# amathislab/HOISDF

Measured on AMD Instinct MI355X. Metric: samples/sec (img + 2048 SDF queries) fwd+bwd at 1/2/4/8 MI355X, higher is better.
Workload: dtype f32 (emulated contractions, f32 accumulate, f16x2 form: operands as scaled hi + lo f16 pieces x 3 products - 22 operand bits, one power-of-two scale per ROW of a linear layer's row operand, per (sample, head) of the attention operands, per weight matrix; the attention backward's dS as three pieces x

## Files before the change

hoisdf_amd/csrc/bnact.hip:

```cpp
#include "common.h"

namespace hoisdf {
namespace {
typedef float f32x4 __attribute__((ext_vector_type(4)));
constexpr int BN_T = 256;

struct Geom { int tpr, rpi; };
__host__ __device__ __forceinline__ Geom geom(int C) { Geom g; g.tpr = C >> 3; g.rpi = BN_T / g.tpr; return g; }
__host__ __device__ __forceinline__ int chunk_of(int C) { return C % 64 == 0 ? 64 : C % 32 == 0 ? 32 : C % 16 == 0 ? 16 : 8; }

__device__ __forceinline__ void ld8(const float* p, float (&v)[8]) {
  const f32x4 a = *reinterpret_cast<const f32x4*>(p), b = *reinterpret_cast<const f32x4*>(p + 4);
  v[0] = a[0]; v[1] = a[1]; v[2] = a[2]; v[3] = a[3]; v[4] = b[0]; v[5] = b[1]; v[6] = b[2]; v[7] = b[3];
}
__device__ __forceinline__ void st8(float* p, const float (&v)[8]) {
  *reinterpret_cast<f32x4*>(p) = f32x4{v[0], v[1], v[2], v[3]};
  *reinterpret_cast<f32x4*>(p + 4) = f32x4{v[4], v[5], v[6], v[7]};
}

__device__ __forceinline__ void block_partials(const float (&s)[16], float* red, int tpr, int rpi, int chunk, float* __restrict__ part) {
  const int tid = threadIdx.x;
#pragma unroll
  for (int j = 0; j < 16; ++j) red[j * BN_T + tid] = s[j];
  __syncthreads();
  float* dst = part + ((size_t)blockIdx.y * gridDim.x + blockIdx.x) * 2 * chunk;
  for (int o = tid; o < 2 * chunk; o += BN_T) {
    const int pl = o / chunk, ch = o - pl * chunk;
    const int j = pl * 8 + (ch & 7), t0 = ch >> 3;
    float a = 0.f;
    for (int g = 0; g < rpi; ++g) a += red[j * BN_T + g * tpr + t0];
    dst[o] = a;
  }
}
__device__ __forceinline__ void sum_partials(const float* __restrict__ part, int S, int chunk, double* dred, double& a1, double& a2) {
  const int tid = threadIdx.x;
  const int lanes = chunk >> 1;
  const int G = BN_T / lanes, lane = tid % lanes, g = tid / lanes;
  const f32x4* src = reinterpret_cast<const f32x4*>(part + (size_t)blockIdx.x * S * 2 * chunk) + lane;
  double acc[4] = {0.0, 0.0, 0.0, 0.0};
  int sl = g;
  for (; sl + 3 * G < S; sl += 4 * G) {
    f32x4 v[4];
#pragma unroll
    for (int u = 0; u < 4; ++u) v[u] = src[(size_t)(sl + u * G) * lanes];
#pragma unroll
    for (int u = 0; u < 4; ++u)
#pragma unroll
      for (int i = 0; i < 4; ++i) acc[i] += (double)v[u][i];
  }
  for (; sl < S; sl += G) {
    const f32x4 v = src[(size_t)sl * lanes];
#pragma unroll
    for (int i = 0; i < 4; ++i) acc[i] += (double)v[i];
  }
#pragma unroll
  for (int i = 0; i < 4; ++i) dred[(g * lanes + lane) * 4 + i] = acc[i];
  __syncthreads();
  a1 = 0.0; a2 = 0.0;
  if (tid < chunk) {
    const int l1 = tid >> 2, l2 = (chunk >> 2) + (tid >> 2), i = tid & 3;
    for (int g2 = 0; g2 < G; ++g2) { a1 += dred[(g2 * lanes + l1) * 4 + i]; a2 += dred[(g2 * lanes + l2) * 4 + i]; }
  }
}

__global__ __launch_bounds__(BN_T) void bn_stats_kernel(const float* __restrict__ x, long ldx, long M, int C, long rows_per_block,
                                                        float* __restrict__ part) {
  __shared__ __attribute__((aligned(16))) float red[16 * BN_T];
  const int chunk = chunk_of(C), tpr = chunk >> 3, rpi = BN_T / tpr;
  const int tid = threadIdx.x, cg = tid % tpr, rg = tid / tpr;
  const int c0 = blockIdx.y * chunk + 8 * cg;
  const long r0 = (long)blockIdx.x * rows_per_block, r1 = r0 + rows_per_block < M ? r0 + rows_per_block : M;
  float s[16], sh[8];
#pragma unroll
  for (int j = 0; j < 16; ++j) s[j] = 0.f;
  ld8(x + c0, sh);
  {
    const long step = rpi;
    long r = r0 + rg;
    for (; r + 3 * step < r1; r += 4 * step) {
      float v[4][8];
#pragma unroll
      for (int u = 0; u < 4; ++u) ld8(x + (r + u * step) * ldx + c0, v[u]);
#pragma unroll
      for (int u = 0; u < 4; ++u)
#pragma unroll
        for (int j = 0; j < 8; ++j) { const float d = v[u][j] - sh[j]; s[j] += d; s[8 + j] = __builtin_fmaf(d, d, s[8 + j]); }
    }
    for (; r < r1; r += step) {
      float v[8];
      ld8(x + r * ldx + c0, v);
#pragma unroll
      for (int j = 0; j < 8; ++j) { const float d = v[j] - sh[j]; s[j] += d; s[8 + j] = __builtin_fmaf(d, d, s[8 + j]); }
    }
  }
  block_partials(s, red, tpr, rpi, chunk, part);
}
__global__ __launch_bounds__(BN_T) void bn_stats_finish_kernel(const float* __restrict__ x, const float* __restrict__ part, int S, long M, int C,
                                                               float* __restrict__ mean, float* __restrict__ invstd, float* __restrict__ run_mean,
                                                               float* __restrict__ run_var, float momentum, float eps) {
  __shared__ __attribute__((aligned(16))) double dred[4 * BN_T];
  const int chunk = chunk_of(C), tid = threadIdx.x;
  double a1, a2;
  sum_partials(part, S, chunk, dred, a1, a2);
  if (tid < chunk) {
    const int c = blockIdx.x * chunk + tid;
    const double m1 = a1 / (double)M;
    const double mu = (double)x[c] + m1;
    double var = a2 / (double)M - m1 * m1;
    var = var > 0.0 ? var : 0.0;
    mean[c] = (float)mu;
    invstd[c] = (float)(1.0 / sqrt(var + (double)eps));
    if (run_mean) run_mean[c] = (float)((1.0 - (double)momentum) * (double)run_mean[c] + (double)momentum * mu);
    if (run_var) run_var[c] = (float)((1.0 - (double)momentum) * (double)run_var[c] + (double)momentum * (M > 1 ? var * (double)M / (double)(M - 1) : var));
  }
}

template <bool RES, bool RELU>
__global__ __launch_bounds__(BN_T) void bn_apply_fwd_kernel(const float* __restrict__ x, long ldx, const float* __restrict__ res, long ldr,
                                                            const float* __restrict__ mean, const float* __restrict__ stat2, int is_var, float eps,
                                                            const float* __restrict__ gamma, const float* __restrict__ beta,
                                                            float* __restrict__ y, uint8_t* __restrict__ bits, long M, int C) {
  const Geom gm = geom(C);
  const int tid = threadIdx.x, cg = tid % gm.tpr, rg = tid / gm.tpr;
  if (rg >= gm.rpi) return;
  float mu[8], k[8], b[8];
  ld8(mean + 8 * cg, mu); ld8(stat2 + 8 * cg, k);
  if (gamma) { float g[8]; ld8(gamma + 8 * cg, g);
#pragma unroll
    for (int j = 0; j < 8; ++j) k[j] = (is_var ? 1.f / sqrtf(k[j] + eps) : k[j]) * g[j];
  } else {
#pragma unroll
    for (int j = 0; j < 8; ++j) k[j] = is_var ? 1.f / sqrtf(k[j] + eps) : k[j];
  }
  if (beta) ld8(beta + 8 * cg, b);
  else {
#pragma unroll
    for (int j = 0; j < 8; ++j) b[j] = 0.f;
  }
  const long step = (long)gridDim.x * gm.rpi;
  for (long r = (long)blockIdx.x * gm.rpi + rg; r < M; r += 4 * step) {
    float v[4][8], q[4][8];
#pragma unroll
    for (int u = 0; u < 4; ++u)
      if (r + u * step < M) { ld8(x + (r + u * step) * ldx + 8 * cg, v[u]); if (RES) ld8(res + (r + u * step) * ldr + 8 * cg, q[u]); }
#pragma unroll
    for (int u = 0; u < 4; ++u) {
      if (r + u * step >= M) break;
      unsigned m = 0u;
#pragma unroll
      for (int j = 0; j < 8; ++j) {
        float t = __builtin_fmaf(v[u][j] - mu[j], k[j], b[j]);
        if (RES) t += q[u][j];
        if (RELU) { m |= (t > 0.f ? 1u : 0u) << j; t = t > 0.f ? t : 0.f; }
        v[u][j] = t;
      }
      st8(y + (r + u * step) * (long)C + 8 * cg, v[u]);
      if (RELU && bits) bits[(r + u * step) * gm.tpr + cg] = (uint8_t)m;
    }
  }
}

template <bool RELU>
__global__ __launch_bounds__(BN_T) void bn_bwd_reduce_kernel(const float* __restrict__ dy, long lddy, const float* __restrict__ x, long ldx,
                                                             const uint8_t* __restrict__ bits, const float* __restrict__ mean,
                                                             long M, int C, long rows_per_block, float* __restrict__ part) {
  __shared__ __attribute__((aligned(16))) float red[16 * BN_T];
  const int chunk = chunk_of(C), tpr = chunk >> 3, rpi = BN_T / tpr;
  const int tid = threadIdx.x, cg = tid % tpr, rg = tid / tpr;
  const int c0 = blockIdx.y * chunk + 8 * cg, b0 = c0 >> 3, ldb = C >> 3;
  const long r0 = (long)blockIdx.x * rows_per_block, r1 = r0 + rows_per_block < M ? r0 + rows_per_block : M;
  float s[16], mu[8];
#pragma unroll
  for (int j = 0; j < 16; ++j) s[j] = 0.f;
  ld8(mean + c0, mu);
  {
    const long step = rpi;
    for (long r = r0 + rg; r < r1; r += 4 * step) {
      float g[4][8], v[4][8]; unsigned m[4];
#pragma unroll
      for (int u = 0; u < 4; ++u)
        if (r + u * step < r1) {
          ld8(dy + (r + u * step) * lddy + c0, g[u]); ld8(x + (r + u * step) * ldx + c0, v[u]);
          m[u] = RELU ? bits[(r + u * step) * ldb + b0] : 0xffu;
        }
#pragma unroll
      for (int u = 0; u < 4; ++u) {
        if (r + u * step >= r1) break;
#pragma unroll
        for (int j = 0; j < 8; ++j) {
          const float gg = (m[u] >> j) & 1u ? g[u][j] : 0.f;
          s[j] += gg; s[8 + j] = __builtin_fmaf(gg, v[u][j] - mu[j], s[8 + j]);
        }
      }
    }
  }
  block_partials(s, red, tpr, rpi, chunk, part);
}
__global__ __launch_bounds__(BN_T) void bn_bwd_finish_kernel(const float* __restrict__ part, int S, long M, int C, const float* __restrict__ invstd,
                                                             float* __restrict__ dgamma, float* __restrict__ dbeta, float* __restrict__ coef) {
  __shared__ __attribute__((aligned(16))) double dred[4 * BN_T];
  const int chunk = chunk_of(C), tid = threadIdx.x;
  double a1, a2;
  sum_partials(part, S, chunk, dred, a1, a2);
  if (tid < chunk) {
    const int c = blockIdx.x * chunk + tid;
    const double is = (double)invstd[c];
    if (dbeta) dbeta[c] = (float)a1;
    if (dgamma) dgamma[c] = (float)(a2 * is);
    coef[c] = (float)(a1 / (double)M);
    coef[C + c] = (float)(a2 * is * is / (double)M);
  }
}

template <bool RES, bool RELU>
__global__ __launch_bounds__(BN_T) void bn_bwd_dx_kernel(const float* __restrict__ dy, long lddy, const float* __restrict__ x, long ldx,
                                                         const uint8_t* __restrict__ bits, const float* __restrict__ mean,
                                                         const float* __restrict__ invstd, const float* __restrict__ gamma,
                                                         const float* __restrict__ coef, float* __restrict__ dx, float* __restrict__ dres,
                                                         long M, int C) {
  const Geom gm = geom(C);
  const int tid = threadIdx.x, cg = tid % gm.tpr, rg = tid / gm.tpr;
  if (rg >= gm.rpi) return;
  float mu[8], k[8], ca[8], cb[8];
  ld8(mean + 8 * cg, mu); ld8(invstd + 8 * cg, k); ld8(coef + 8 * cg, ca); ld8(coef + C + 8 * cg, cb);
  if (gamma) { float g[8]; ld8(gamma + 8 * cg, g);
#pragma unroll
    for (int j = 0; j < 8; ++j) k[j] *= g[j];
  }
  const long step = (long)gridDim.x * gm.rpi;
  for (long r = (long)blockIdx.x * gm.rpi + rg; r < M; r += 4 * step) {
    float g[4][8], v[4][8]; unsigned m[4];
#pragma unroll
    for (int u = 0; u < 4; ++u)
      if (r + u * step < M) {
        ld8(dy + (r + u * step) * lddy + 8 * cg, g[u]); ld8(x + (r + u * step) * ldx + 8 * cg, v[u]);
        m[u] = RELU ? bits[(r + u * step) * gm.tpr + cg] : 0xffu;
      }
#pragma unroll
    for (int u = 0; u < 4; ++u) {
      if (r + u * step >= M) break;
#pragma unroll
      for (int j = 0; j < 8; ++j) {
        const float gg = (m[u] >> j) & 1u ? g[u][j] : 0.f;
        g[u][j] = gg;
        v[u][j] = k[j] * (gg - ca[j] - (v[u][j] - mu[j]) * cb[j]);
      }
      st8(dx + (r + u * step) * (long)C + 8 * cg, v[u]);
      if (RES) st8(dres + (r + u * step) * (long)C + 8 * cg, g[u]);
    }
  }
}

inline bool shape_ok(long M, int C, long ld) { return M > 0 && C >= 8 && C % 8 == 0 && C <= 8 * BN_T && ld >= C && ld % 4 == 0; }
inline bool al16(const void* p) { return (reinterpret_cast<uintptr_t>(p) & 15) == 0; }
inline void reduce_grid(long M, int C, long& rows_per_block, int& slices, int& chunks) {
  const int chunk = chunk_of(C), rpi = BN_T / (chunk >> 3);
  chunks = C / chunk;
  int smax = 1024 / chunks;
  smax = smax < 16 ? 16 : smax > 256 ? 256 : smax;
  const long unit = (long)rpi * 4;
  const long k = (M + unit * smax - 1) / (unit * smax);
  rows_per_block = unit * (k < 1 ? 1 : k);
  slices = cdiv(M, rows_per_block);
}
inline int stream_grid(long M, int C) {
  const Geom gm = geom(C);
  const long it = (M + gm.rpi - 1) / gm.rpi;
  long g = (it + 3) / 4;
  return (int)(g < 1 ? 1 : g > 4096 ? 4096 : g);
}
}
}

using namespace hoisdf;

extern "C" long hoisdf_bn_workspace_floats(long M, int C) {
  if (!shape_ok(M, C, C)) return 0;
  long rpb; int slices, chunks;
  reduce_grid(M, C, rpb, slices, chunks);
  return (long)slices * 2 * C + 2L * C;
}

extern "C" int hoisdf_bn_stats(const float* x, long ldx, long M, int C, float* mean, float* invstd, float* running_mean, float* running_var,
                               float momentum, float eps, float* workspace, long workspace_floats, void* stream) {
  HOISDF_REQUIRE(x && mean && invstd && workspace, HOISDF_ERR_INVALID, "bn_stats: null pointer");
  HOISDF_REQUIRE(shape_ok(M, C, ldx) && al16(x) && al16(mean) && al16(invstd), HOISDF_ERR_INVALID,
                 "bn_stats: M=%ld C=%d ld=%ld (C %% 8 == 0, C <= %d, 16-byte aligned rows)", M, C, ldx, 8 * BN_T);
  HOISDF_REQUIRE(workspace_floats >= hoisdf_bn_workspace_floats(M, C), HOISDF_ERR_WORKSPACE, "bn_stats: workspace of %ld floats, need %ld",
                 workspace_floats, hoisdf_bn_workspace_floats(M, C));
  long rpb; int slices, chunks;
  reduce_grid(M, C, rpb, slices, chunks);
  hipLaunchKernelGGL(bn_stats_kernel, dim3(slices, chunks), dim3(BN_T), 0, as_stream(stream), x, ldx, M, C, rpb, workspace);
  hipLaunchKernelGGL(bn_stats_finish_kernel, dim3(chunks), dim3(BN_T), 0, as_stream(stream), x, workspace, slices, M, C, mean, invstd, running_mean,
                     running_var, momentum, eps);
  return check_launch("bn_stats");
}

extern "C" int hoisdf_bn_apply_fwd(const float* x, long ldx, const float* residual, long ldr, const float* mean, const float* invstd_or_var,
                                   int second_is_variance, float eps, const float* gamma, const float* beta, int relu, float* y,
                                   uint8_t* sign_bits, long M, int C, void* stream) {
  HOISDF_REQUIRE(x && mean && invstd_or_var && y, HOISDF_ERR_INVALID, "bn_apply_fwd: null pointer");
  HOISDF_REQUIRE(shape_ok(M, C, ldx) && (!residual || (shape_ok(M, C, ldr) && al16(residual))) && al16(x) && al16(y) && al16(mean) &&
                     al16(invstd_or_var) && (!gamma || al16(gamma)) && (!beta || al16(beta)),
                 HOISDF_ERR_INVALID, "bn_apply_fwd: M=%ld C=%d ld=%ld (C %% 8 == 0, C <= %d, 16-byte aligned rows)", M, C, ldx, 8 * BN_T);
  const dim3 grid(stream_grid(M, C)), block(BN_T);
  hipStream_t st = as_stream(stream);
#define BN_FWD(RES_, RELU_) hipLaunchKernelGGL((bn_apply_fwd_kernel<RES_, RELU_>), grid, block, 0, st, x, ldx, residual, ldr, mean, invstd_or_var, \
                                               second_is_variance, eps, gamma, beta, y, sign_bits, M, C)
  if (residual) { if (relu) BN_FWD(true, true); else BN_FWD(true, false); }
  else { if (relu) BN_FWD(false, true); else BN_FWD(false, false); }
#undef BN_FWD
  return check_launch("bn_apply_fwd");
}

extern "C" int hoisdf_bn_bwd(const float* dy, long lddy, const float* x, long ldx, const uint8_t* sign_bits, const float* mean,
                             const float* invstd, const float* gamma, float* dx, float* d_residual, float* dgamma, float* dbeta, long M, int C,
                             float* workspace, long workspace_floats, void* stream) {
  HOISDF_REQUIRE(dy && x && mean && invstd && dx && workspace, HOISDF_ERR_INVALID, "bn_bwd: null pointer");
  HOISDF_REQUIRE(shape_ok(M, C, ldx) && shape_ok(M, C, lddy) && al16(dy) && al16(x) && al16(dx) && al16(mean) && al16(invstd) &&
                     (!gamma || al16(gamma)) && (!d_residual || al16(d_residual)) && al16(workspace),
                 HOISDF_ERR_INVALID, "bn_bwd: M=%ld C=%d ldx=%ld lddy=%ld (C %% 8 == 0, C <= %d, 16-byte aligned rows)", M, C, ldx, lddy, 8 * BN_T);
  HOISDF_REQUIRE(workspace_floats >= hoisdf_bn_workspace_floats(M, C), HOISDF_ERR_WORKSPACE, "bn_bwd: workspace of %ld floats, need %ld",
                 workspace_floats, hoisdf_bn_workspace_floats(M, C));
  long rpb; int slices, chunks;
  reduce_grid(M, C, rpb, slices, chunks);
  float* coef = workspace + (long)slices * 2 * C;
  hipStream_t st = as_stream(stream);
  if (sign_bits) hipLaunchKernelGGL((bn_bwd_reduce_kernel<true>), dim3(slices, chunks), dim3(BN_T), 0, st, dy, lddy, x, ldx, sign_bits, mean, M, C, rpb,
                                    workspace);
  else hipLaunchKernelGGL((bn_bwd_reduce_kernel<false>), dim3(slices, chunks), dim3(BN_T), 0, st, dy, lddy, x, ldx, sign_bits, mean, M, C, rpb, workspace);
  hipLaunchKernelGGL(bn_bwd_finish_kernel, dim3(chunks), dim3(BN_T), 0, st, workspace, slices, M, C, invstd, dgamma, dbeta, coef);
  if (int rc = check_launch("bn_bwd (reduce)")) return rc;
  const dim3 grid(stream_grid(M, C)), block(BN_T);
#define BN_DX(RES_, RELU_) hipLaunchKernelGGL((bn_bwd_dx_kernel<RES_, RELU_>), grid, block, 0, st, dy, lddy, x, ldx, sign_bits, mean, invstd, gamma, coef, \
                                              dx, d_residual, M, C)
  if (d_residual) { if (sign_bits) BN_DX(true, true); else BN_DX(true, false); }
  else { if (sign_bits) BN_DX(false, true); else BN_DX(false, false); }
#undef BN_DX
  return check_launch("bn_bwd (dx)");
}
```

Baseline: 444.9.

## Fuse BN backward finish into reduce kernel via last-block arrival tickets

The batch-norm backward reduction now has the last-arriving block of each channel chunk, detected with an atomic ticket counter, sum all slice partials and compute dgamma, dbeta and the coefficients. This removes the separate finish kernel launch. The partial-sum loop also gains a 16-way unrolled path for more loads in flight. The cost is atomic stores and fences, a per-stream ticket array kept in a host-side map, and a serial tail where one block per chunk does the final sum.

```diff
diff --git a/hoisdf_amd/csrc/bnact.hip b/hoisdf_amd/csrc/bnact.hip
--- a/hoisdf_amd/csrc/bnact.hip
+++ b/hoisdf_amd/csrc/bnact.hip
@@ -1,9 +1,14 @@
+#include <map>
+#include <mutex>
+#include <utility>
+
 #include "common.h"
 
 namespace hoisdf {
 namespace {
 typedef float f32x4 __attribute__((ext_vector_type(4)));
 constexpr int BN_T = 256;
+constexpr int FLAG_WORD = 16 * BN_T - 1;
 
 struct Geom { int tpr, rpi; };
 __host__ __device__ __forceinline__ Geom geom(int C) { Geom g; g.tpr = C >> 3; g.rpi = BN_T / g.tpr; return g; }
@@ -18,7 +23,8 @@
   *reinterpret_cast<f32x4*>(p + 4) = f32x4{v[4], v[5], v[6], v[7]};
 }
 
-__device__ __forceinline__ void block_partials(const float (&s)[16], float* red, int tpr, int rpi, int chunk, float* __restrict__ part) {
+template <bool THROUGH>
+__device__ __forceinline__ void block_partials(const float (&s)[16], float* red, int tpr, int rpi, int chunk, float* part) {
   const int tid = threadIdx.x;
 #pragma unroll
   for (int j = 0; j < 16; ++j) red[j * BN_T + tid] = s[j];
@@ -29,16 +35,42 @@
     const int j = pl * 8 + (ch & 7), t0 = ch >> 3;
     float a = 0.f;
     for (int g = 0; g < rpi; ++g) a += red[j * BN_T + g * tpr + t0];
-    dst[o] = a;
-  }
-}
-__device__ __forceinline__ void sum_partials(const float* __restrict__ part, int S, int chunk, double* dred, double& a1, double& a2) {
+    if (THROUGH) __hip_atomic_store(dst + o, a, __ATOMIC_RELAXED, __HIP_MEMORY_SCOPE_AGENT);
+    else dst[o] = a;
+  }
+}
+__device__ __forceinline__ bool chunk_complete(unsigned* __restrict__ tickets, unsigned* flag) {
+  asm volatile("s_waitcnt vmcnt(0)" ::: "memory");
+  __syncthreads();
+  if (threadIdx.x == 0) {
+    unsigned* t = tickets + blockIdx.y;
+    const bool last = __hip_atomic_fetch_add(t, 1u, __ATOMIC_RELAXED, __HIP_MEMORY_SCOPE_AGENT) == gridDim.x - 1;
+    if (last) {
+      __builtin_amdgcn_fence(__ATOMIC_ACQUIRE, "agent");
+      asm volatile("s_waitcnt vmcnt(0)" ::: "memory");
+      __hip_atomic_store(t, 0u, __ATOMIC_RELAXED, __HIP_MEMORY_SCOPE_AGENT);
+    }
+    *flag = last ? 1u : 0u;
+  }
+  __syncthreads();
+  return *flag != 0u;
+}
+__device__ __forceinline__ void sum_partials(const float* part, int S, int chunk, double* dred, double& a1, double& a2) {
   const int tid = threadIdx.x;
   const int lanes = chunk >> 1;
   const int G = BN_T / lanes, lane = tid % lanes, g = tid / lanes;
-  const f32x4* src = reinterpret_cast<const f32x4*>(part + (size_t)blockIdx.x * S * 2 * chunk) + lane;
+  const f32x4* src = reinterpret_cast<const f32x4*>(part + (size_t)blockIdx.y * S * 2 * chunk) + lane;
   double acc[4] = {0.0, 0.0, 0.0, 0.0};
   int sl = g;
+  for (; sl + 15 * G < S; sl += 16 * G) {
+    f32x4 v[16];
+#pragma unroll
+    for (int u = 0; u < 16; ++u) v[u] = src[(size_t)(sl + u * G) * lanes];
+#pragma unroll
+    for (int u = 0; u < 16; ++u)
+#pragma unroll
+      for (int i = 0; i < 4; ++i) acc[i] += (double)v[u][i];
+  }
   for (; sl + 3 * G < S; sl += 4 * G) {
     f32x4 v[4];
 #pragma unroll
@@ -93,7 +125,7 @@
       for (int j = 0; j < 8; ++j) { const float d = v[j] - sh[j]; s[j] += d; s[8 + j] = __builtin_fmaf(d, d, s[8 + j]); }
     }
   }
-  block_partials(s, red, tpr, rpi, chunk, part);
+  block_partials<false>(s, red, tpr, rpi, chunk, part);
 }
 __global__ __launch_bounds__(BN_T) void bn_stats_finish_kernel(const float* __restrict__ x, const float* __restrict__ part, int S, long M, int C,
                                                                float* __restrict__ mean, float* __restrict__ invstd, float* __restrict__ run_mean,
@@ -103,7 +135,7 @@
   double a1, a2;
   sum_partials(part, S, chunk, dred, a1, a2);
   if (tid < chunk) {
-    const int c = blockIdx.x * chunk + tid;
+    const int c = blockIdx.y * chunk + tid;
     const double m1 = a1 / (double)M;
     const double mu = (double)x[c] + m1;
     double var = a2 / (double)M - m1 * m1;
@@ -163,7 +195,9 @@
 template <bool RELU>
 __global__ __launch_bounds__(BN_T) void bn_bwd_reduce_kernel(const float* __restrict__ dy, long lddy, const float* __restrict__ x, long ldx,
                                                              const uint8_t* __restrict__ bits, const float* __restrict__ mean,
-                                                             long M, int C, long rows_per_block, float* __restrict__ part) {
+                                                             long M, int C, long rows_per_block, float* part, unsigned* __restrict__ tickets,
+                                                             const float* __restrict__ invstd, float* __restrict__ dgamma,
+                                                             float* __restrict__ dbeta, float* __restrict__ coef) {
   __shared__ __attribute__((aligned(16))) float red[16 * BN_T];
   const int chunk = chunk_of(C), tpr = chunk >> 3, rpi = BN_T / tpr;
   const int tid = threadIdx.x, cg = tid % tpr, rg = tid / tpr;
@@ -194,16 +228,12 @@
       }
     }
   }
-  block_partials(s, red, tpr, rpi, chunk, part);
-}
-__global__ __launch_bounds__(BN_T) void bn_bwd_finish_kernel(const float* __restrict__ part, int S, long M, int C, const float* __restrict__ invstd,
-                                                             float* __restrict__ dgamma, float* __restrict__ dbeta, float* __restrict__ coef) {
-  __shared__ __attribute__((aligned(16))) double dred[4 * BN_T];
-  const int chunk = chunk_of(C), tid = threadIdx.x;
+  block_partials<true>(s, red, tpr, rpi, chunk, part);
+  if (!chunk_complete(tickets, reinterpret_cast<unsigned*>(red) + FLAG_WORD)) return;
   double a1, a2;
-  sum_partials(part, S, chunk, dred, a1, a2);
+  sum_partials(part, gridDim.x, chunk, reinterpret_cast<double*>(red), a1, a2);
   if (tid < chunk) {
-    const int c = blockIdx.x * chunk + tid;
+    const int c = blockIdx.y * chunk + tid;
     const double is = (double)invstd[c];
     if (dbeta) dbeta[c] = (float)a1;
     if (dgamma) dgamma[c] = (float)(a2 * is);
@@ -263,6 +293,21 @@
   rows_per_block = unit * (k < 1 ? 1 : k);
   slices = cdiv(M, rows_per_block);
 }
+unsigned* bn_tickets(hipStream_t st) {
+  static std::mutex mu;
+  static std::map<std::pair<int, hipStream_t>, unsigned*> arrays;
+  int dev = 0;
+  if (hipGetDevice(&dev) != hipSuccess) return nullptr;
+  std::lock_guard<std::mutex> lk(mu);
+  unsigned*& t = arrays[std::make_pair(dev, st)];
+  if (!t) {
+    unsigned* p = nullptr;
+    if (hipMalloc(reinterpret_cast<void**>(&p), BN_T * sizeof(unsigned)) != hipSuccess) return nullptr;
+    if (hipMemsetAsync(p, 0, BN_T * sizeof(unsigned), st) != hipSuccess) { (void)hipFree(p); return nullptr; }
+    t = p;
+  }
+  return t;
+}
 inline int stream_grid(long M, int C) {
   const Geom gm = geom(C);
   const long it = (M + gm.rpi - 1) / gm.rpi;
@@ -284,14 +329,14 @@
 extern "C" int hoisdf_bn_stats(const float* x, long ldx, long M, int C, float* mean, float* invstd, float* running_mean, float* running_var,
                                float momentum, float eps, float* workspace, long workspace_floats, void* stream) {
   HOISDF_REQUIRE(x && mean && invstd && workspace, HOISDF_ERR_INVALID, "bn_stats: null pointer");
-  HOISDF_REQUIRE(shape_ok(M, C, ldx) && al16(x) && al16(mean) && al16(invstd), HOISDF_ERR_INVALID,
+  HOISDF_REQUIRE(shape_ok(M, C, ldx) && al16(x) && al16(mean) && al16(invstd) && al16(workspace), HOISDF_ERR_INVALID,
                  "bn_stats: M=%ld C=%d ld=%ld (C %% 8 == 0, C <= %d, 16-byte aligned rows)", M, C, ldx, 8 * BN_T);
   HOISDF_REQUIRE(workspace_floats >= hoisdf_bn_workspace_floats(M, C), HOISDF_ERR_WORKSPACE, "bn_stats: workspace of %ld floats, need %ld",
                  workspace_floats, hoisdf_bn_workspace_floats(M, C));
   long rpb; int slices, chunks;
   reduce_grid(M, C, rpb, slices, chunks);
   hipLaunchKernelGGL(bn_stats_kernel, dim3(slices, chunks), dim3(BN_T), 0, as_stream(stream), x, ldx, M, C, rpb, workspace);
-  hipLaunchKernelGGL(bn_stats_finish_kernel, dim3(chunks), dim3(BN_T), 0, as_stream(stream), x, workspace, slices, M, C, mean, invstd, running_mean,
+  hipLaunchKernelGGL(bn_stats_finish_kernel, dim3(1, chunks), dim3(BN_T), 0, as_stream(stream), x, workspace, slices, M, C, mean, invstd, running_mean,
                      running_var, momentum, eps);
   return check_launch("bn_stats");
 }
@@ -326,10 +371,12 @@
   reduce_grid(M, C, rpb, slices, chunks);
   float* coef = workspace + (long)slices * 2 * C;
   hipStream_t st = as_stream(stream);
+  unsigned* tickets = bn_tickets(st);
+  HOISDF_REQUIRE(tickets, HOISDF_ERR_LAUNCH, "bn_bwd: cannot allocate the arrival counters");
   if (sign_bits) hipLaunchKernelGGL((bn_bwd_reduce_kernel<true>), dim3(slices, chunks), dim3(BN_T), 0, st, dy, lddy, x, ldx, sign_bits, mean, M, C, rpb,
-                                    workspace);
-  else hipLaunchKernelGGL((bn_bwd_reduce_kernel<false>), dim3(slices, chunks), dim3(BN_T), 0, st, dy, lddy, x, ldx, sign_bits, mean, M, C, rpb, workspace);
-  hipLaunchKernelGGL(bn_bwd_finish_kernel, dim3(chunks), dim3(BN_T), 0, st, workspace, slices, M, C, invstd, dgamma, dbeta, coef);
+                                    workspace, tickets, invstd, dgamma, dbeta, coef);
+  else hipLaunchKernelGGL((bn_bwd_reduce_kernel<false>), dim3(slices, chunks), dim3(BN_T), 0, st, dy, lddy, x, ldx, sign_bits, mean, M, C, rpb, workspace,
+                          tickets, invstd, dgamma, dbeta, coef);
   if (int rc = check_launch("bn_bwd (reduce)")) return rc;
   const dim3 grid(stream_grid(M, C)), block(BN_T);
 #define BN_DX(RES_, RELU_) hipLaunchKernelGGL((bn_bwd_dx_kernel<RES_, RELU_>), grid, block, 0, st, dy, lddy, x, ldx, sign_bits, mean, invstd, gamma, coef, \
```

Result: no change. 444.6 (-0.1%).
